# mikemey/cellcomm

Measured on NVIDIA B200. Metric: BiGAN train cells/sec, higher is better.
Workload: dtype bf16

## Files before the change

cellcomm_b200/csrc/gemm_sm100.cu:

```cuda
#include <cuda.h>

#include <mutex>
#include <unordered_map>

#include "common.cuh"

namespace cc {

constexpr int BM = 128;
constexpr int BK = 64;
constexpr int UMMA_K = 16;
constexpr int MAX_SEG = CC_GEMM_MAX_SEG;

struct EpiParams {
  int M, N;
  float alpha;
  const float* bias;
  int act;
  const bf16* dact_y;
  long long ld_dact;
  int dact;
  bf16* out16;
  long long ld16;
  int beta16;
// ... 884 lines not shown
      const int nkb_u = unit_nkb(u);
      int seg = 0, kb_in_seg = unit_kb0(u);
      while (seg < p.nseg - 1 && kb_in_seg >= p.kblocks[seg]) {
        kb_in_seg -= p.kblocks[seg];
        ++seg;
      }
      for (int i = 0; i < nkb_u; ++i, ++it) {
        const int s = it % STAGES;
        const uint32_t ph = (it / STAGES) & 1u;
        mbar_wait(empty_bar(s), ph ^ 1u, 11);
        if (elect_one()) {
          const uint32_t a_dst = smem_base + s * STAGE_BYTES;
          const uint32_t b_dst = a_dst + A_BYTES;
          const int k0 = kb_in_seg * BK;
          mbar_expect_tx(full_bar(s), p.stage_tx);
          if (RMS_DIRECT && A_MN && B_MN && keep != 0) {
#pragma unroll
            for (int j = 0; j < BM / 64; ++j)
              tma_load_2d_pol(a_dst + j * (64 * BK * 2), &maps.a[seg], full_bar(s), m0 + 64 * j, k0,
                              keep);
#pragma unroll
            for (int j = 0; j < BN / 64; ++j) {
              if (j >= p.b_boxes) continue;
              if (CLUSTER == 2) {
                if ((j & 1) == rank)
                  tma_load_2d_mc_pol(b_dst + j * (64 * BK * 2), &maps.b[seg], full_bar(s),
                                     n0 + 64 * j, k0, (uint16_t)3, keep);
              } else {
                tma_load_2d_pol(b_dst + j * (64 * BK * 2), &maps.b[seg], full_bar(s), n0 + 64 * j,
                                k0, keep);
              }
            }
          } else if (A_MN) {
#pragma unroll
            for (int j = 0; j < BM / 64; ++j)
              tma_load_2d(a_dst + j * (64 * BK * 2), &maps.a[seg], full_bar(s), m0 + 64 * j, k0);
          } else {
            tma_load_2d(a_dst, &maps.a[seg], full_bar(s), k0, m0);
          }
          if (RMS_DIRECT && A_MN && B_MN && keep != 0) {
          } else if (CLUSTER == 2) {
            if (B_MN) {
#pragma unroll
              for (int j = 0; j < BN / 64; ++j)
                if (j < p.b_boxes && (j & 1) == rank)
                  tma_load_2d_mc(b_dst + j * (64 * BK * 2), &maps.b[seg], full_bar(s), n0 + 64 * j,
                                 k0, (uint16_t)3);
            } else {
              tma_load_2d_mc(b_dst + rank * p.b_half_rows * (BK * 2), &maps.b[seg], full_bar(s), k0,
                             n0 + rank * p.b_half_rows, (uint16_t)3);
            }
          } else if (B_MN) {
#pragma unroll
            for (int j = 0; j < BN / 64; ++j)
              if (j < p.b_boxes)
                tma_load_2d(b_dst + j * (64 * BK * 2), &maps.b[seg], full_bar(s), n0 + 64 * j, k0);
          } else {
            tma_load_2d(b_dst, &maps.b[seg], full_bar(s), k0, n0);
          }
        }
        __syncwarp();
        if (++kb_in_seg >= p.kblocks[seg] && seg < p.nseg - 1) {
          kb_in_seg = 0;
          ++seg;
        }
      }
    }
  } else if (warp == 1) {
    uint32_t it = 0, tl = 0;
    for (int u = unit0; (!PAIR || rank == 0) && u < num_units; u += unit_step, ++tl) {
      const uint32_t acc = tl & 1u, aph = (tl >> 1) & 1u;
      mbar_wait(tempty_bar(acc), aph ^ 1u, 12);
      tcgen05_fence_after();
      const uint32_t d_tmem = tmem_acc + acc * BN;
      const int nkb = unit_nkb(u);
      for (int i = 0; i < nkb; ++i, ++it) {
        const int s = it % STAGES;
        const uint32_t ph = (it / STAGES) & 1u;
        mbar_wait(full_bar(s), ph, 13);
        tcgen05_fence_after();
        if (elect_one()) {
          const uint32_t a_src = smem_base + s * STAGE_BYTES;
          const uint32_t b_src = a_src + A_BYTES;
#pragma unroll
          for (int k = 0; k < BK / UMMA_K; ++k) {
            const uint64_t adesc = p.adesc_hi | (uint64_t)(((a_src + k * p.a_kstep) & 0x3FFFFu) >> 4);
            const uint64_t bdesc = p.bdesc_hi | (uint64_t)(((b_src + k * p.b_kstep) & 0x3FFFFu) >> 4);
            if (PAIR) umma_bf16_pair(d_tmem, adesc, bdesc, p.idesc, (i > 0 || k > 0) ? 1u : 0u);
            else umma_bf16(d_tmem, adesc, bdesc, p.idesc, (i > 0 || k > 0) ? 1u : 0u);
          }
          if (PAIR) {
            umma_commit_pair(empty_bar(s), (uint16_t)3);
            if (i == nkb - 1) umma_commit_pair(tfull_bar(acc), (uint16_t)3);
          } else {
            if (CLUSTER == 2) umma_commit_mc(empty_bar(s), (uint16_t)3);
            else umma_commit(empty_bar(s));
            if (i == nkb - 1) umma_commit(tfull_bar(acc));
          }
        }
        __syncwarp();
      }
    }
  } else {
    const int q = warp & 3;
    const int ew = warp - 2;
    constexpr int COLS_PER_WARP = BN / (EPI_WARPS / 4);
    const int col_lo = (ew >> 2) * COLS_PER_WARP;
    uint32_t tl = 0;
    for (int u = unit0; u < num_units; u += unit_step, ++tl) {
      const int m0 = unit_m0(u), n0 = unit_n0(u);
      const uint32_t acc = tl & 1u, aph = (tl >> 1) & 1u;
      mbar_wait(tfull_bar(acc), aph, 14);
      tcgen05_fence_after();
      const uint32_t t_row = tmem_acc + ((uint32_t)(q * 32) << 16) + acc * BN;
      if (m0 < p.epi.M) {
#pragma unroll 1
        for (int c = col_lo; c < col_lo + COLS_PER_WARP; c += 32) {
          if (c >= p.bn_eff || n0 + c >= p.epi.N) break;
          uint32_t raw[32];
          tmem_ld32(t_row + (uint32_t)c, raw);
          tmem_ld_wait();
          if constexpr (RMS_DIRECT) rms_blocked_chunk(p.epi, lane, m0 + q * 32, n0 + c, raw);
          else epilogue_chunk<MATH>(p.epi, epi_stage + ew * (32 * EPI_LD), lane, m0 + q * 32, n0 + c, raw,
                                    (long long)unit_split(u) * p.partial_stride);
        }
      }
      tcgen05_fence_before();
      __syncwarp();
      if (lane == 0) {
        if (PAIR) mbar_arrive_cluster(mapa_cluster(tempty_bar(acc), 0));
        else mbar_arrive(tempty_bar(acc));
      }
    }
  }
  tcgen05_fence_before();
  __syncthreads();
  if (CLUSTER == 2) cluster_sync_all();
  if (warp == 1) {
    if (PAIR)
      asm volatile("tcgen05.dealloc.cta_group::2.sync.aligned.b32 %0, %1;" ::"r"(tmem_acc),
                   "r"(TMEM_COLS)
                   : "memory");
    else
      asm volatile("tcgen05.dealloc.cta_group::1.sync.aligned.b32 %0, %1;" ::"r"(tmem_acc),
                   "r"(TMEM_COLS)
                   : "memory");
  }
}

}
#include "wgrad_rmsprop_kernel.cuh"
namespace cc {

__global__ void splitk_finalize_kernel(const EpiParams e, const float* __restrict__ partial,
                                       long long partial_ld, long long partial_stride, int splits) {
  const int groups = (e.N + 3) / 4;
  const long long idx = (long long)blockIdx.x * blockDim.x + threadIdx.x;
  if (idx >= (long long)e.M * groups) return;
  const int r = (int)(idx / groups);
  const int c0 = (int)(idx % groups) * 4;
  const float* src = partial + (long long)r * partial_ld + c0;
  float4 a = make_float4(0.f, 0.f, 0.f, 0.f);
  for (int s0 = 0; s0 < splits; s0 += 8) {
    float4 q[8];
#pragma unroll
    for (int u = 0; u < 8; ++u)
      q[u] = (s0 + u < splits)
                 ? __ldcs(reinterpret_cast<const float4*>(src + (long long)(s0 + u) * partial_stride))
                 : make_float4(0.f, 0.f, 0.f, 0.f);
#pragma unroll
    for (int u = 0; u < 8; ++u) {
      if (s0 + u < splits) {
        a.x += q[u].x;
        a.y += q[u].y;
        a.z += q[u].z;
        a.w += q[u].w;
      }
    }
  }
  float v[4] = {a.x, a.y, a.z, a.w};
  const int ncols = min(4, e.N - c0);
#pragma unroll
  for (int j = 0; j < 4; ++j) {
    float x = v[j] * e.alpha;
    if (e.bias != nullptr && j < ncols) x += __ldg(e.bias + c0 + j);
    if (e.act == CC_ACT_SIGMOID) x = sigmoidf_(x);
    else if (e.act == CC_ACT_RELU) x = fmaxf(x, 0.f);
    v[j] = x;
  }
  if (e.dact != 0) {
    const bf16* yrow = e.dact_y + (long long)r * e.ld_dact + c0;
#pragma unroll
    for (int j = 0; j < 4; ++j) {
      if (j < ncols) {
        const float y = bf2f(yrow[j]);
        v[j] *= (e.dact == CC_ACT_SIGMOID) ? y * (1.f - y) : (y > 0.f ? 1.f : 0.f);
      }
    }
  }
  if (e.out32 != nullptr) {
    float* o = e.out32 + (long long)r * e.ld32 + c0;
    if (ncols == 4 && (((uintptr_t)o) & 15) == 0 && !e.beta32) {
      *reinterpret_cast<float4*>(o) = make_float4(v[0], v[1], v[2], v[3]);
    } else {
#pragma unroll
      for (int j = 0; j < 4; ++j)
        if (j < ncols) o[j] = e.beta32 ? o[j] + v[j] : v[j];
    }
  }
  if (e.out16 != nullptr) {
    bf16* o = e.out16 + (long long)r * e.ld16 + c0;
    if (ncols == 4 && (((uintptr_t)o) & 7) == 0 && !e.beta16) {
      __nv_bfloat162 p0 = __floats2bfloat162_rn(v[0], v[1]);
      __nv_bfloat162 p1 = __floats2bfloat162_rn(v[2], v[3]);
      uint2 u;
      u.x = *reinterpret_cast<uint32_t*>(&p0);
      u.y = *reinterpret_cast<uint32_t*>(&p1);
      *reinterpret_cast<uint2*>(o) = u;
    } else {
#pragma unroll
      for (int j = 0; j < 4; ++j)
        if (j < ncols) o[j] = f2bf(e.beta16 ? bf2f(o[j]) + v[j] : v[j]);
    }
    if (e.out16_lo != nullptr) {
      bf16* l = e.out16_lo + (long long)r * e.ld16_lo + c0;
#pragma unroll
      for (int j = 0; j < 4; ++j)
        if (j < ncols) l[j] = f2bf(v[j] - bf2f(f2bf(v[j])));
    }
  }
}

typedef CUresult (*PFN_encodeTiled)(CUtensorMap*, CUtensorMapDataType, cuuint32_t, void*,
                                    const cuuint64_t*, const cuuint64_t*, const cuuint32_t*,
                                    const cuuint32_t*, CUtensorMapInterleave, CUtensorMapSwizzle,
                                    CUtensorMapL2promotion, CUtensorMapFloatOOBfill);

static PFN_encodeTiled get_encode_fn() {
  static PFN_encodeTiled fn = nullptr;
  static std::once_flag once;
  std::call_once(once, [] {
    void* ptr = nullptr;
    cudaDriverEntryPointQueryResult qres;
    if (cudaGetDriverEntryPoint("cuTensorMapEncodeTiled", &ptr, cudaEnableDefault, &qres) ==
            cudaSuccess &&
        qres == cudaDriverEntryPointSuccess)
      fn = (PFN_encodeTiled)ptr;
  });
  return fn;
}

struct MapKey {
  const void* ptr;
  uint64_t inner, outer, ld;
  uint32_t box_inner, box_outer;
  uint32_t kind;
  bool operator==(const MapKey& o) const {
    return ptr == o.ptr && inner == o.inner && outer == o.outer && ld == o.ld &&
           box_inner == o.box_inner && box_outer == o.box_outer && kind == o.kind;
  }
};
struct MapKeyHash {
  size_t operator()(const MapKey& k) const {
    uint64_t h = (uint64_t)(uintptr_t)k.ptr * 0x9E3779B97F4A7C15ull;
    h ^= k.inner + 0x9E3779B97F4A7C15ull + (h << 6) + (h >> 2);
    h ^= k.outer + 0x9E3779B97F4A7C15ull + (h << 6) + (h >> 2);
    h ^= k.ld + 0x9E3779B97F4A7C15ull + (h << 6) + (h >> 2);
    h ^= ((uint64_t)k.box_inner << 32 | k.box_outer) + 0x9E3779B97F4A7C15ull + (h << 6) + (h >> 2);
    h ^= k.kind + 0x9E3779B97F4A7C15ull + (h << 6) + (h >> 2);
    return (size_t)h;
  }
};

enum MapKind : uint32_t {
  MAP_BF16_SW128 = 0,
  MAP_F32_SW128 = 1,
  MAP_BF16_SW64 = 2,
  MAP_F32_SW128_L2_256 = 3
};

static int make_map_kind(CUtensorMap* out, const void* ptr, uint64_t inner, uint64_t outer,
                         uint64_t ld, uint32_t box_inner, uint32_t box_outer, MapKind kind) {
  static std::mutex mu;
  static std::unordered_map<MapKey, CUtensorMap, MapKeyHash> cache;
  MapKey key{ptr, inner, outer, ld, box_inner, box_outer, (uint32_t)kind};
  {
    std::lock_guard<std::mutex> g(mu);
    auto it = cache.find(key);
    if (it != cache.end()) {
      *out = it->second;
      return 0;
    }
  }
  const bool f32 = kind == MAP_F32_SW128 || kind == MAP_F32_SW128_L2_256;
  const uint64_t esize = f32 ? 4 : 2;
  PFN_encodeTiled enc = get_encode_fn();
  CC_REQUIRE(enc != nullptr, "cuTensorMapEncodeTiled is unavailable (no CUDA driver?)");
  CC_REQUIRE(((uintptr_t)ptr & 15) == 0, "cc_gemm: operand base %p is not 16-byte aligned", ptr);
  CC_REQUIRE((ld * esize) % 16 == 0, "cc_gemm: operand ld=%llu is not a multiple of 16 bytes",
             (unsigned long long)ld);
  CC_REQUIRE(inner > 0 && outer > 0, "cc_gemm: empty operand");
  cuuint64_t dims[2] = {inner, outer};
  cuuint64_t strides[1] = {ld * esize};
  cuuint32_t box[2] = {box_inner, box_outer};
  cuuint32_t estr[2] = {1, 1};
  CUresult r = enc(out,
                   f32 ? CU_TENSOR_MAP_DATA_TYPE_FLOAT32 : CU_TENSOR_MAP_DATA_TYPE_BFLOAT16,
                   2, const_cast<void*>(ptr), dims, strides, box, estr,
                   CU_TENSOR_MAP_INTERLEAVE_NONE,
                   kind == MAP_BF16_SW64 ? CU_TENSOR_MAP_SWIZZLE_64B : CU_TENSOR_MAP_SWIZZLE_128B,
                   (kind == MAP_BF16_SW128 || kind == MAP_F32_SW128_L2_256)
                       ? CU_TENSOR_MAP_L2_PROMOTION_L2_256B
                       : CU_TENSOR_MAP_L2_PROMOTION_L2_128B,
                   CU_TENSOR_MAP_FLOAT_OOB_FILL_NONE);
  CC_REQUIRE(r == CUDA_SUCCESS,
             "cuTensorMapEncodeTiled failed (%d) ptr=%p inner=%llu outer=%llu ld=%llu box=%ux%u",
             (int)r, ptr, (unsigned long long)inner, (unsigned long long)outer,
             (unsigned long long)ld, box_inner, box_outer);
  {
    std::lock_guard<std::mutex> g(mu);
    if (cache.size() > (1u << 16)) cache.clear();
    cache.emplace(key, *out);
  }
  return 0;
}

static int make_map(CUtensorMap* out, const void* ptr, uint64_t inner, uint64_t outer, uint64_t ld,
                    uint32_t box_inner, uint32_t box_outer) {
  return make_map_kind(out, ptr, inner, outer, ld, box_inner, box_outer, MAP_BF16_SW128);
}

static uint64_t desc_hi(uint32_t lbo_bytes, uint32_t sbo_bytes) {
  uint64_t d = 0;
  d |= (uint64_t)((lbo_bytes >> 4) & 0x3FFF) << 16;
  d |= (uint64_t)((sbo_bytes >> 4) & 0x3FFF) << 32;
  d |= (uint64_t)1 << 46;
  d |= (uint64_t)2 << 61;
  return d;
}

static int env_int(const char* name, int dflt) {
  const char* v = getenv(name);
  return v ? atoi(v) : dflt;
}

struct GemmEnv {
  int sms;
  int bn;
  int splits;
  int persistent;
  int cluster;
  int rms_cluster;
  int bn_eff;
  int mn_lbo;
  int mn_sbo;
  int mn_kstep;
  int k_lbo;
  int k_sbo;
  int rms_cs;
  int rms_warps;
  int rms_nfast;
  int rms_tma;
  int rms_p16_tma;
  int rms_interleave;
  int rms_pair;
  int pair;
  int rms_l2_256;
  int rms_keep;
  int persistent_splitk;
};
static GemmEnv g_env;
static std::atomic<int> g_env_state{0};
static std::mutex g_env_mu;
static int g_num_sms = 0;

static const GemmEnv& gemm_env() {
  if (g_env_state.load(std::memory_order_acquire) == 0) {
    std::lock_guard<std::mutex> lock(g_env_mu);
    GemmEnv e;
    e.sms = env_int("CC_GEMM_SMS", 0);
    e.bn = env_int("CC_GEMM_BN", 0);
    e.splits = env_int("CC_GEMM_SPLITS", 0);
    e.persistent = env_int("CC_GEMM_PERSISTENT", 1);
    e.cluster = env_int("CC_GEMM_CLUSTER", 2);
    e.rms_cluster = env_int("CC_GEMM_RMS_CLUSTER", -1);
    e.bn_eff = env_int("CC_GEMM_BN_EFF", 0);
    e.mn_lbo = env_int("CC_GEMM_MN_LBO", 64 * BK * 2);
    e.mn_sbo = env_int("CC_GEMM_MN_SBO", 1024);
    e.mn_kstep = env_int("CC_GEMM_MN_KSTEP", UMMA_K * 128);
    e.k_lbo = env_int("CC_GEMM_K_LBO", 16);
    e.k_sbo = env_int("CC_GEMM_K_SBO", 1024);
    e.rms_cs = env_int("CC_GEMM_RMS_CS", 1);
    e.rms_warps = env_int("CC_GEMM_RMS_WARPS", 8);
    e.rms_nfast = env_int("CC_GEMM_RMS_NFAST", -1);
    e.rms_tma = env_int("CC_GEMM_RMS_TMA", -1);
    e.rms_p16_tma = env_int("CC_GEMM_RMS_P16_TMA", 0);
    e.rms_interleave = env_int("CC_GEMM_RMS_INTERLEAVE", 1);
    e.rms_pair = env_int("CC_GEMM_RMS_PAIR", 0);
    e.pair = env_int("CC_GEMM_PAIR", 0);
    e.rms_l2_256 = env_int("CC_GEMM_RMS_L2_256", 0);
    e.rms_keep = env_int("CC_GEMM_RMS_KEEP_OPERANDS", 0);
    e.persistent_splitk = env_int("CC_GEMM_PERSISTENT_SPLITK", 1);
    g_env = e;
    g_env_state.store(1, std::memory_order_release);
  }
  return g_env;
}

template <int BN, int STAGES>
static constexpr size_t smem_bytes() {
  return (size_t)STAGES * (BM * BK * 2 + BN * BK * 2) + 8 * (2 * STAGES + 2) + 1024;
}

template <int BN, int STAGES, bool A_MN, bool B_MN>
static int launch_cfg(const TmaMaps& maps, const GemmParams& p, dim3 grid, cudaStream_t st) {
  auto kern = gemm_tcgen05_kernel<BN, STAGES, A_MN, B_MN>;
  static bool attr_set = false;
  constexpr size_t smem = smem_bytes<BN, STAGES>();
  if (!attr_set) {
    CC_CHECK_CUDA(cudaFuncSetAttribute(kern, cudaFuncAttributeMaxDynamicSharedMemorySize, (int)smem));
    attr_set = true;
  }
  kern<<<grid, 128, smem, st>>>(maps, p);
  CC_CHECK_LAUNCH();
  return 0;
}

template <int BN, int STAGES>
static int launch_major(const TmaMaps& maps, const GemmParams& p, dim3 grid, bool a_mn, bool b_mn,
                        cudaStream_t st) {
  if (!a_mn && b_mn) return launch_cfg<BN, STAGES, false, true>(maps, p, grid, st);
  if (!a_mn && !b_mn) return launch_cfg<BN, STAGES, false, false>(maps, p, grid, st);
  if (a_mn && b_mn) return launch_cfg<BN, STAGES, true, true>(maps, p, grid, st);
  return launch_cfg<BN, STAGES, true, false>(maps, p, grid, st);
}

template <int BN, int STAGES, int EPI_WARPS, bool PAIR = false, bool RMS_DIRECT = false>
static constexpr size_t smem_bytes_persistent() {
  return (size_t)STAGES * (BM * BK * 2 + (PAIR ? BN / 2 : BN) * BK * 2) + 8 * (2 * STAGES + 6) + 16 +
         (RMS_DIRECT ? 0 : EPI_WARPS * 32 * EPI_LD * 4) + 1024;
}

template <int BN, int STAGES, bool A_MN, bool B_MN, bool MATH, int EPI_WARPS, bool N_FAST, int CLUSTER,
          bool PAIR = false, bool RMS_DIRECT = false>
static int launch_persistent_one(const TmaMaps& maps, const GemmParams& p, int mt, int nt,
                                 int num_sms, cudaStream_t st) {
  auto kern = gemm_tcgen05_persistent_kernel<BN, STAGES, A_MN, B_MN, MATH, EPI_WARPS, N_FAST, CLUSTER,
                                             PAIR, RMS_DIRECT>;
  static bool attr_set = false;
  static int max_ctas = 0;
  constexpr size_t smem = smem_bytes_persistent<BN, STAGES, EPI_WARPS, PAIR, RMS_DIRECT>();
  static_assert(smem <= 232448, "shared memory per CTA");
  constexpr int threads = 64 + 32 * EPI_WARPS;
  if (!attr_set) {
    CC_CHECK_CUDA(cudaFuncSetAttribute(kern, cudaFuncAttributeMaxDynamicSharedMemorySize, (int)smem));
    max_ctas = num_sms;
    if (CLUSTER > 1) {
      cudaLaunchConfig_t q{};
      q.gridDim = dim3((unsigned)(num_sms / CLUSTER * CLUSTER));
      q.blockDim = dim3(threads);
      q.dynamicSmemBytes = smem;
      cudaLaunchAttribute qa[1];
      qa[0].id = cudaLaunchAttributeClusterDimension;
      qa[0].val.clusterDim.x = CLUSTER;
      qa[0].val.clusterDim.y = 1;
      qa[0].val.clusterDim.z = 1;
      q.attrs = qa;
      q.numAttrs = 1;
      int nclusters = 0;
      CC_CHECK_CUDA(cudaOccupancyMaxActiveClusters(&nclusters, kern, &q));
      CC_REQUIRE(nclusters >= 1, "cc_gemm: no %d-CTA cluster fits on this device", CLUSTER);
      if (nclusters * CLUSTER < max_ctas) max_ctas = nclusters * CLUSTER;
    }
    attr_set = true;
  }
  const int units = ((mt + CLUSTER - 1) / CLUSTER) * nt * (p.psplits > 1 ? p.psplits : 1);
  int grid = units * CLUSTER < max_ctas ? units * CLUSTER : max_ctas / CLUSTER * CLUSTER;
  cudaLaunchConfig_t cfg{};
  cfg.gridDim = dim3((unsigned)grid);
  cfg.blockDim = dim3(threads);
  cfg.dynamicSmemBytes = smem;
  cfg.stream = st;
  cudaLaunchAttribute attr[1];
  attr[0].id = cudaLaunchAttributeClusterDimension;
  attr[0].val.clusterDim.x = CLUSTER;
  attr[0].val.clusterDim.y = 1;
  attr[0].val.clusterDim.z = 1;
  cfg.attrs = attr;
  cfg.numAttrs = 1;
  CC_CHECK_CUDA(cudaLaunchKernelEx(&cfg, kern, maps, p, mt, nt));
  count_launch();
  return 0;
}

template <int BN, int STAGES, int EPI_WARPS>
static constexpr int pair_stages() {
  return BN == 256 ? (EPI_WARPS == 8 ? 5 : 6) : STAGES;
}

template <int BN, int STAGES, bool A_MN, bool B_MN, bool MATH, int EPI_WARPS = 4, bool N_FAST = false>
static int launch_persistent_cfg(const TmaMaps& maps, const GemmParams& p, int mt, int nt,
                                 int num_sms, cudaStream_t st) {
  if (BN == 256 && p.cluster == 2 && p.pair)
    return launch_persistent_one<BN, pair_stages<BN, STAGES, EPI_WARPS>(), A_MN, B_MN, MATH, EPI_WARPS,
                                 N_FAST, 2, BN == 256>(maps, p, mt, nt, num_sms, st);
  if (p.cluster == 2)
    return launch_persistent_one<BN, STAGES, A_MN, B_MN, MATH, EPI_WARPS, N_FAST, 2>(maps, p, mt, nt, num_sms, st);
  return launch_persistent_one<BN, STAGES, A_MN, B_MN, MATH, EPI_WARPS, N_FAST, 1>(maps, p, mt, nt, num_sms, st);
}

template <int BN, int STAGES, bool MATH>
static int launch_persistent_m(const TmaMaps& maps, const GemmParams& p, int mt, int nt,
                               int num_sms, bool a_mn, bool b_mn, cudaStream_t st) {
  if (!a_mn && b_mn) return launch_persistent_cfg<BN, STAGES, false, true, MATH>(maps, p, mt, nt, num_sms, st);
  if (!a_mn && !b_mn) return launch_persistent_cfg<BN, STAGES, false, false, MATH>(maps, p, mt, nt, num_sms, st);
  if (a_mn && b_mn) return launch_persistent_cfg<BN, STAGES, true, true, MATH>(maps, p, mt, nt, num_sms, st);
  return launch_persistent_cfg<BN, STAGES, true, false, MATH>(maps, p, mt, nt, num_sms, st);
}

template <int BN, int STAGES>
static int launch_persistent(const TmaMaps& maps, const GemmParams& p, int mt, int nt, int num_sms,
                             bool a_mn, bool b_mn, cudaStream_t st) {
  const EpiParams& e = p.epi;
  const bool math = e.alpha != 1.f || e.bias != nullptr || e.act != 0 || e.dact != 0;
  if (math) return launch_persistent_m<BN, STAGES, true>(maps, p, mt, nt, num_sms, a_mn, b_mn, st);
  return launch_persistent_m<BN, STAGES, false>(maps, p, mt, nt, num_sms, a_mn, b_mn, st);
}

template <bool N_FAST, int CLUSTER, bool PAIR = false>
static int launch_rms_tma(const RmsMaps& maps, const GemmParams& p, int mt, int nt, int num_sms,
                          cudaStream_t st) {
  static_assert(!PAIR || CLUSTER == 2, "the CTA pair is a cluster of two");
  void (*kern)(const RmsMaps, const GemmParams, const int, const int);
  if (PAIR) kern = wgrad_rmsprop_pair_kernel<N_FAST>;
  else kern = wgrad_rmsprop_tma_kernel<N_FAST, CLUSTER>;
  static bool attr_set = false;
  static int max_ctas = 0;
  constexpr size_t smem = PAIR ? RMSP_SMEM_BYTES : RMS_SMEM_BYTES;
  constexpr int threads = 64 + 32 * RMS_EPI_WARPS;
  if (!attr_set) {
    CC_CHECK_CUDA(cudaFuncSetAttribute(kern, cudaFuncAttributeMaxDynamicSharedMemorySize, (int)smem));
    max_ctas = num_sms;
    if (CLUSTER > 1) {
      cudaLaunchConfig_t q{};
      q.gridDim = dim3((unsigned)(num_sms / CLUSTER * CLUSTER));
      q.blockDim = dim3(threads);
      q.dynamicSmemBytes = smem;
      cudaLaunchAttribute qa[1];
      qa[0].id = cudaLaunchAttributeClusterDimension;
      qa[0].val.clusterDim.x = CLUSTER;
      qa[0].val.clusterDim.y = 1;
      qa[0].val.clusterDim.z = 1;
      q.attrs = qa;
      q.numAttrs = 1;
      int nclusters = 0;
      CC_CHECK_CUDA(cudaOccupancyMaxActiveClusters(&nclusters, kern, &q));
      CC_REQUIRE(nclusters >= 1, "cc_gemm: no %d-CTA cluster fits on this device", CLUSTER);
      if (nclusters * CLUSTER < max_ctas) max_ctas = nclusters * CLUSTER;
    }
    attr_set = true;
  }
  const int units = ((mt + CLUSTER - 1) / CLUSTER) * nt;
  int grid = units * CLUSTER < max_ctas ? units * CLUSTER : max_ctas / CLUSTER * CLUSTER;
  cudaLaunchConfig_t cfg{};
  cfg.gridDim = dim3((unsigned)grid);
  cfg.blockDim = dim3(threads);
  cfg.dynamicSmemBytes = smem;
  cfg.stream = st;
  cudaLaunchAttribute attr[1];
  attr[0].id = cudaLaunchAttributeClusterDimension;
  attr[0].val.clusterDim.x = CLUSTER;
  attr[0].val.clusterDim.y = 1;
  attr[0].val.clusterDim.z = 1;
  cfg.attrs = attr;
  cfg.numAttrs = 1;
  CC_CHECK_CUDA(cudaLaunchKernelEx(&cfg, kern, maps, p, mt, nt));
  count_launch();
  return 0;
}

int gemm_impl(const cc_gemm_desc* d, cudaStream_t st) {
  const GemmEnv& ENV = gemm_env();
  CC_REQUIRE(d != nullptr, "cc_gemm: null descriptor");
  CC_REQUIRE(d->M > 0 && d->N > 0, "cc_gemm: empty output %dx%d", d->M, d->N);
  CC_REQUIRE(d->nseg >= 1 && d->nseg <= MAX_SEG, "cc_gemm: nseg=%d out of range", d->nseg);
  CC_REQUIRE(d->out16 != nullptr || d->out32 != nullptr || d->rms_p32 != nullptr,
             "cc_gemm: no output");
  CC_REQUIRE(d->rms_p32 == nullptr || (d->rms_ms != nullptr && d->rms_mom != nullptr),
             "cc_gemm: fused RMSprop needs ms and mom");
  CC_REQUIRE(d->route_world >= 0 && d->route_world <= CC_PEER_MAX, "cc_gemm: route_world=%d",
             d->route_world);
  CC_REQUIRE(d->out16_lo == nullptr || (d->out16 != nullptr && d->beta16 == 0),
             "cc_gemm: out16_lo needs a plain out16 (the high-order term)");
  if (d->rms_blocked) {
    CC_REQUIRE(d->rms_p32 != nullptr && d->a_mn_major && d->b_mn_major && d->N > 128 &&
                   d->alpha == 1.f && d->bias == nullptr && d->act == 0 && d->dact_y == nullptr &&
                   d->out16 == nullptr && d->beta32 == 0 && d->route_world == 0 &&
                   d->force_splits <= 1 && (d->force_bn == 0 || d->force_bn == 256),
               "cc_gemm: rms_blocked is for plain weight-gradient GEMMs (X^T dZ, N > 128)");
    CC_REQUIRE(d->rms_row0 >= 0 && (d->rms_ld & 31) == 0 &&
                   ((((uintptr_t)d->rms_p32) | ((uintptr_t)d->rms_ms) | ((uintptr_t)d->rms_mom) |
                     ((uintptr_t)d->rms_p16) | ((uintptr_t)d->rms_p16_lo) | ((uintptr_t)d->out32)) & 15) == 0 &&
                   (d->out32 == nullptr || (d->ld32 & 3) == 0),
               "cc_gemm: rms_blocked needs 16-byte aligned blocks, rms_ld %% 32 == 0 (rms_ld=%lld)",
               (long long)d->rms_ld);
  }
  CC_REQUIRE(d->rms_p16_lo == nullptr || d->rms_blocked,
             "cc_gemm: rms_p16_lo is written by the blocked fused-optimiser epilogue only");
  if (d->route_world > 0) {
    CC_REQUIRE(d->out32 != nullptr && d->beta32 == 0 && d->workspace == nullptr &&
                   d->rms_p32 == nullptr,
               "cc_gemm: a routed output needs a plain fp32 output without split-K");
    CC_REQUIRE(d->route_shard > 0 && (d->route_shard & 7) == 0 && d->route_shard < (1ll << 32) &&
                   d->route_off0 >= 0 && (d->route_off0 & 3) == 0,
               "cc_gemm: route_shard=%lld route_off0=%lld", (long long)d->route_shard,
               (long long)d->route_off0);
    for (int q = 0; q < d->route_world; ++q)
      CC_REQUIRE(d->route_base[q] != nullptr, "cc_gemm: route_base[%d] is null", q);
  }
  if (g_num_sms == 0) {
    int dev = 0;
    CC_CHECK_CUDA(cudaGetDevice(&dev));
    CC_CHECK_CUDA(cudaDeviceGetAttribute(&g_num_sms, cudaDevAttrMultiProcessorCount, dev));
    const int cap = ENV.sms;
    if (cap >= 2 && cap < g_num_sms) g_num_sms = cap / 2 * 2;
  }
  const bool a_mn = d->a_mn_major != 0, b_mn = d->b_mn_major != 0;

  int bn = d->force_bn ? d->force_bn : ENV.bn;
  if (bn == 0) bn = (d->N > 128) ? 256 : 128;
  CC_REQUIRE(bn == 128 || bn == 256, "cc_gemm: BN=%d unsupported", bn);

  GemmParams p{};
  TmaMaps maps;
  memset(&maps, 0, sizeof(maps));
  p.nseg = d->nseg;
  int total = 0;
  for (int s = 0; s < d->nseg; ++s) {
    CC_REQUIRE(d->k[s] > 0, "cc_gemm: segment %d has k=%d", s, d->k[s]);
    p.kblocks[s] = (d->k[s] + BK - 1) / BK;
    total += p.kblocks[s];
  }
  p.total_kblocks = total;

  const int mt = (d->M + BM - 1) / BM;
  int nt = (d->N + bn - 1) / bn;
  int splits = 1;
  const long long Mpad = (long long)mt * BM, Npad = (long long)nt * bn;
  if (d->workspace != nullptr && d->rms_p32 == nullptr) {
    int want = d->force_splits ? d->force_splits : ENV.splits;
    if (want == 0) {
      const int tiles = mt * nt;
      if (2 * tiles <= g_num_sms && total >= 8) {
        want = (2 * g_num_sms) / tiles;
        if (want < 1) want = 1;
        if (want > total / 4) want = total / 4;
      } else {
        want = 1;
      }
    }
    if (want > total) want = total;
    const long long cap = d->workspace_elems / (Mpad * Npad);
    if (want > cap) want = (int)cap;
    if (want >= 2) splits = want;
  }
  p.kb_per_split = (total + splits - 1) / splits;
  splits = (total + p.kb_per_split - 1) / p.kb_per_split;
  if (splits >= 2) {
    p.partial = d->workspace;
    p.partial_ld = Npad;
    p.partial_stride = Mpad * Npad;
  } else {
    p.partial = nullptr;
    p.kb_per_split = total;
    splits = 1;
  }
  const bool psk = splits >= 2 && ENV.persistent != 0 && ENV.persistent_splitk != 0;
  const bool persistent =
      (splits == 1 || psk) && (ENV.persistent != 0 || d->rms_p32 != nullptr ||
                               d->route_world > 0);

  const bool rms_cluster = ENV.rms_cluster < 0 ? total > 8 : ENV.rms_cluster != 0;
  p.cluster = (persistent && mt >= 2 && ENV.cluster == 2 &&
               (d->rms_p32 == nullptr || rms_cluster)) ? 2 : 1;
  int bn_eff = bn;
  if (persistent && bn == 256 && d->rms_p32 == nullptr && splits == 1) {
    const int forced = ENV.bn_eff;
    if (forced >= 32 && forced <= 256 && forced % 32 == 0) {
      bn_eff = forced;
    } else {
      long long best = -1;
      const int mu = (mt + p.cluster - 1) / p.cluster, slots = g_num_sms / p.cluster;
      for (int cand = 256; cand >= 128; cand -= 64) {
        const long long units = (long long)mu * ((d->N + cand - 1) / cand);
        const long long cost = ((units + slots - 1) / slots) * (cand + 128);
        if (best < 0 || cost < best) {
          best = cost;
          bn_eff = cand;
        }
      }
    }
    nt = (d->N + bn_eff - 1) / bn_eff;
  }
  p.bn_eff = bn_eff;
  p.b_boxes = (bn_eff + 63) / 64;
  p.b_half_rows = bn_eff / 2;
  p.stage_tx = (unsigned)(BM * BK * 2 + (b_mn ? p.b_boxes * 64 * BK * 2 : bn_eff * BK * 2));
  p.pair = (p.cluster == 2 && bn == 256 && ENV.pair != 0 && splits == 1 &&
            (b_mn ? bn_eff % 128 == 0 : bn_eff % 32 == 0)) ? 1 : 0;
  if (p.pair) {
    p.b_boxes = bn_eff / 128;
    p.stage_tx = (unsigned)(BM * BK * 2 + (bn_eff / 2) * BK * 2);
  }

  for (int s = 0; s < d->nseg; ++s) {
    int rc;
    if (a_mn)
      rc = make_map(&maps.a[s], d->a[s], (uint64_t)d->M, (uint64_t)d->k[s], (uint64_t)d->lda[s], 64, BK);
    else
      rc = make_map(&maps.a[s], d->a[s], (uint64_t)d->k[s], (uint64_t)d->M, (uint64_t)d->lda[s], BK, BM);
    if (rc) return rc;
    if (b_mn)
      rc = make_map(&maps.b[s], d->b[s], (uint64_t)d->N, (uint64_t)d->k[s], (uint64_t)d->ldb[s], 64, BK);
    else
      rc = make_map(&maps.b[s], d->b[s], (uint64_t)d->k[s], (uint64_t)d->N, (uint64_t)d->ldb[s], BK,
                    (uint32_t)(persistent ? (p.cluster == 2 ? bn_eff / 2 : bn_eff) : bn));
    if (rc) return rc;
  }

  const uint32_t mn_lbo = (uint32_t)ENV.mn_lbo;
  const uint32_t mn_sbo = (uint32_t)ENV.mn_sbo;
  const uint32_t mn_kstep = (uint32_t)ENV.mn_kstep;
  const uint32_t k_lbo = (uint32_t)ENV.k_lbo;
  const uint32_t k_sbo = (uint32_t)ENV.k_sbo;
  p.adesc_hi = a_mn ? desc_hi(mn_lbo, mn_sbo) : desc_hi(k_lbo, k_sbo);
  p.bdesc_hi = b_mn ? desc_hi(mn_lbo, mn_sbo) : desc_hi(k_lbo, k_sbo);
  p.a_kstep = a_mn ? mn_kstep : UMMA_K * 2;
  p.b_kstep = b_mn ? mn_kstep : UMMA_K * 2;
  p.idesc = (1u << 4) | (1u << 7) | (1u << 10) | ((a_mn ? 1u : 0u) << 15) |
            ((b_mn ? 1u : 0u) << 16) | ((uint32_t)((persistent ? bn_eff : bn) >> 3) << 17) |
            ((uint32_t)(((persistent && p.pair) ? 2 * BM : BM) >> 4) << 24);

  EpiParams& e = p.epi;
  e.M = d->M;
  e.N = d->N;
  e.alpha = d->alpha;
  e.bias = d->bias;
  e.act = d->act;
  e.dact_y = (const bf16*)d->dact_y;
  e.ld_dact = d->ld_dact;
  e.dact = d->dact_y ? d->dact : 0;
  e.out16 = (bf16*)d->out16;
  e.ld16 = d->ld16;
  e.beta16 = d->beta16;
  e.out16_lo = (bf16*)d->out16_lo;
  e.ld16_lo = d->ld16_lo;
  e.out32 = d->out32;
  e.ld32 = d->ld32;
  e.beta32 = d->beta32;
  e.rms_p32 = d->rms_p32;
  e.rms_ms = d->rms_ms;
  e.rms_mom = d->rms_mom;
  e.rms_p16 = (bf16*)d->rms_p16;
  e.rms_ld = d->rms_ld;
  e.rms_lr = d->rms_lr;
  e.rms_rho = d->rms_rho;
  e.rms_momentum = d->rms_momentum;
  e.rms_eps = d->rms_eps;
  e.rms_cs = (ENV.rms_cs ? 1 : 0) | (ENV.rms_l2_256 ? 8 : 0);
  e.rms_blocked = d->rms_blocked;
  e.rms_row0 = d->rms_row0;
  e.rms_p16lo = d->rms_blocked ? (bf16*)d->rms_p16_lo : nullptr;
  e.rms_keep_operands = ENV.rms_keep;
  e.route_world = d->route_world;
  e.route_shard = (unsigned)d->route_shard;
  e.route_off0 = d->route_off0;
  for (int q = 0; q < CC_PEER_MAX; ++q)
    e.route_base[q] = q < d->route_world ? d->route_base[q] : nullptr;

  if (persistent) {
// ... 118 lines not shown
```

Before: 58550.

## Add mma.sync small-GEMM path with split-K for small shapes

Adds a cp.async and ldmatrix based mma.sync kernel with 64x64 tiles, a 4-stage pipeline and optional split-K, and routes small or skinny GEMMs to it by default instead of the tcgen05/TMA kernel. The goal is to avoid the fixed setup cost and poor SM fill of the large-tile UMMA path on small problems. It also moves the split-K finalize epilogue into a shared templated helper. The risk is that the shape heuristic sends some GEMMs to a slower legacy tensor-core path.

```diff
diff --git a/cellcomm_b200/csrc/gemm_sm100.cu b/cellcomm_b200/csrc/gemm_sm100.cu
--- a/cellcomm_b200/csrc/gemm_sm100.cu
+++ b/cellcomm_b200/csrc/gemm_sm100.cu
@@ -1060,6 +1060,67 @@
 #include "wgrad_rmsprop_kernel.cuh"
 namespace cc {
 
+template <int NC>
+__device__ __forceinline__ void epilogue_store_cols(const EpiParams& e, int r, int c0, float (&v)[NC]) {
+  const int ncols = min(NC, e.N - c0);
+#pragma unroll
+  for (int j = 0; j < NC; ++j) {
+    float x = v[j] * e.alpha;
+    if (e.bias != nullptr && j < ncols) x += __ldg(e.bias + c0 + j);
+    if (e.act == CC_ACT_SIGMOID) x = sigmoidf_(x);
+    else if (e.act == CC_ACT_RELU) x = fmaxf(x, 0.f);
+    v[j] = x;
+  }
+  if (e.dact != 0) {
+    const bf16* yrow = e.dact_y + (long long)r * e.ld_dact + c0;
+#pragma unroll
+    for (int j = 0; j < NC; ++j) {
+      if (j < ncols) {
+        const float y = bf2f(yrow[j]);
+        v[j] *= (e.dact == CC_ACT_SIGMOID) ? y * (1.f - y) : (y > 0.f ? 1.f : 0.f);
+      }
+    }
+  }
+  if (e.out32 != nullptr) {
+    float* o = e.out32 + (long long)r * e.ld32 + c0;
+    if (ncols == NC && (((uintptr_t)o) & (4 * NC - 1)) == 0 && !e.beta32) {
+      if constexpr (NC == 4)
+        *reinterpret_cast<float4*>(o) = make_float4(v[0], v[1], v[2], v[3]);
+      else
+        *reinterpret_cast<float2*>(o) = make_float2(v[0], v[1]);
+    } else {
+#pragma unroll
+      for (int j = 0; j < NC; ++j)
+        if (j < ncols) o[j] = e.beta32 ? o[j] + v[j] : v[j];
+    }
+  }
+  if (e.out16 != nullptr) {
+    bf16* o = e.out16 + (long long)r * e.ld16 + c0;
+    if (ncols == NC && (((uintptr_t)o) & (2 * NC - 1)) == 0 && !e.beta16) {
+      __nv_bfloat162 p0 = __floats2bfloat162_rn(v[0], v[1]);
+      if constexpr (NC == 4) {
+        __nv_bfloat162 p1 = __floats2bfloat162_rn(v[2], v[3]);
+        uint2 u;
+        u.x = *reinterpret_cast<uint32_t*>(&p0);
+        u.y = *reinterpret_cast<uint32_t*>(&p1);
+        *reinterpret_cast<uint2*>(o) = u;
+      } else {
+        *reinterpret_cast<__nv_bfloat162*>(o) = p0;
+      }
+    } else {
+#pragma unroll
+      for (int j = 0; j < NC; ++j)
+        if (j < ncols) o[j] = f2bf(e.beta16 ? bf2f(o[j]) + v[j] : v[j]);
+    }
+    if (e.out16_lo != nullptr) {
+      bf16* l = e.out16_lo + (long long)r * e.ld16_lo + c0;
+#pragma unroll
+      for (int j = 0; j < NC; ++j)
+        if (j < ncols) l[j] = f2bf(v[j] - bf2f(f2bf(v[j])));
+    }
+  }
+}
+
 __global__ void splitk_finalize_kernel(const EpiParams e, const float* __restrict__ partial,
                                        long long partial_ld, long long partial_stride, int splits) {
   const int groups = (e.N + 3) / 4;
@@ -1087,56 +1148,163 @@
     }
   }
   float v[4] = {a.x, a.y, a.z, a.w};
-  const int ncols = min(4, e.N - c0);
-#pragma unroll
-  for (int j = 0; j < 4; ++j) {
-    float x = v[j] * e.alpha;
-    if (e.bias != nullptr && j < ncols) x += __ldg(e.bias + c0 + j);
-    if (e.act == CC_ACT_SIGMOID) x = sigmoidf_(x);
-    else if (e.act == CC_ACT_RELU) x = fmaxf(x, 0.f);
-    v[j] = x;
-  }
-  if (e.dact != 0) {
-    const bf16* yrow = e.dact_y + (long long)r * e.ld_dact + c0;
-#pragma unroll
-    for (int j = 0; j < 4; ++j) {
-      if (j < ncols) {
-        const float y = bf2f(yrow[j]);
-        v[j] *= (e.dact == CC_ACT_SIGMOID) ? y * (1.f - y) : (y > 0.f ? 1.f : 0.f);
-      }
-    }
-  }
-  if (e.out32 != nullptr) {
-    float* o = e.out32 + (long long)r * e.ld32 + c0;
-    if (ncols == 4 && (((uintptr_t)o) & 15) == 0 && !e.beta32) {
-      *reinterpret_cast<float4*>(o) = make_float4(v[0], v[1], v[2], v[3]);
+  epilogue_store_cols<4>(e, r, c0, v);
+}
+
+constexpr int SG_BM = 64, SG_BN = 64, SG_BK = 32, SG_STAGES = 4, SG_THREADS = 128;
+constexpr int SG_TILE = 64 * (SG_BK + 8);
+
+struct SmallGemmParams {
+  EpiParams epi;
+  const bf16* a[MAX_SEG];
+  const bf16* b[MAX_SEG];
+  long long lda[MAX_SEG], ldb[MAX_SEG];
+  int k[MAX_SEG];
+  int kblocks[MAX_SEG];
+  int nseg, total_kblocks, kb_per_split;
+  float* partial;
+  long long partial_ld, partial_stride;
+};
+
+__device__ __forceinline__ void cp_async16(uint32_t dst, const void* src, int bytes) {
+  asm volatile("cp.async.cg.shared.global [%0], [%1], 16, %2;" ::"r"(dst), "l"(src), "r"(bytes)
+               : "memory");
+}
+__device__ __forceinline__ void ldsm_x4(uint32_t addr, uint32_t (&r)[4]) {
+  asm volatile("ldmatrix.sync.aligned.m8n8.x4.shared.b16 {%0, %1, %2, %3}, [%4];"
+               : "=r"(r[0]), "=r"(r[1]), "=r"(r[2]), "=r"(r[3])
+               : "r"(addr));
+}
+__device__ __forceinline__ void ldsm_x4_t(uint32_t addr, uint32_t (&r)[4]) {
+  asm volatile("ldmatrix.sync.aligned.m8n8.x4.trans.shared.b16 {%0, %1, %2, %3}, [%4];"
+               : "=r"(r[0]), "=r"(r[1]), "=r"(r[2]), "=r"(r[3])
+               : "r"(addr));
+}
+__device__ __forceinline__ void mma_bf16_16816(float (&c)[4], const uint32_t (&a)[4], uint32_t b0,
+                                               uint32_t b1) {
+  asm volatile(
+      "mma.sync.aligned.m16n8k16.row.col.f32.bf16.bf16.f32 {%0, %1, %2, %3}, {%4, %5, %6, %7}, "
+      "{%8, %9}, {%0, %1, %2, %3};"
+      : "+f"(c[0]), "+f"(c[1]), "+f"(c[2]), "+f"(c[3])
+      : "r"(a[0]), "r"(a[1]), "r"(a[2]), "r"(a[3]), "r"(b0), "r"(b1));
+}
+
+template <bool MN_MAJOR>
+__device__ __forceinline__ void sg_load_tile(uint32_t dst, const bf16* base, long long ld, int i0,
+                                             int outer_n, int k0, int kn) {
+#pragma unroll
+  for (int q = 0; q < 2; ++q) {
+    const int c = threadIdx.x + q * SG_THREADS;
+    int valid, sidx;
+    long long off;
+    if (MN_MAJOR) {
+      const int row = c >> 3, col = (c & 7) * 8;
+      const int gk = k0 + row, gi = i0 + col;
+      valid = gk < kn ? min(max(outer_n - gi, 0), 8) : 0;
+      off = (long long)gk * ld + gi;
+      sidx = row * (SG_BM + 8) + col;
     } else {
-#pragma unroll
-      for (int j = 0; j < 4; ++j)
-        if (j < ncols) o[j] = e.beta32 ? o[j] + v[j] : v[j];
-    }
-  }
-  if (e.out16 != nullptr) {
-    bf16* o = e.out16 + (long long)r * e.ld16 + c0;
-    if (ncols == 4 && (((uintptr_t)o) & 7) == 0 && !e.beta16) {
-      __nv_bfloat162 p0 = __floats2bfloat162_rn(v[0], v[1]);
-      __nv_bfloat162 p1 = __floats2bfloat162_rn(v[2], v[3]);
-      uint2 u;
-      u.x = *reinterpret_cast<uint32_t*>(&p0);
-      u.y = *reinterpret_cast<uint32_t*>(&p1);
-      *reinterpret_cast<uint2*>(o) = u;
-    } else {
-#pragma unroll
-      for (int j = 0; j < 4; ++j)
-        if (j < ncols) o[j] = f2bf(e.beta16 ? bf2f(o[j]) + v[j] : v[j]);
-    }
-    if (e.out16_lo != nullptr) {
-      bf16* l = e.out16_lo + (long long)r * e.ld16_lo + c0;
-#pragma unroll
-      for (int j = 0; j < 4; ++j)
-        if (j < ncols) l[j] = f2bf(v[j] - bf2f(f2bf(v[j])));
-    }
-  }
+      const int row = c >> 2, col = (c & 3) * 8;
+      const int gi = i0 + row, gk = k0 + col;
+      valid = gi < outer_n ? min(max(kn - gk, 0), 8) : 0;
+      off = (long long)gi * ld + gk;
+      sidx = row * (SG_BK + 8) + col;
+    }
+    cp_async16(dst + 2u * (uint32_t)sidx, valid > 0 ? (const void*)(base + off) : (const void*)base,
+               valid * 2);
+  }
+}
+
+template <bool A_MN, bool B_MN>
+__global__ void __launch_bounds__(SG_THREADS) gemm_small_kernel(const SmallGemmParams p) {
+  __shared__ __align__(128) bf16 sa[SG_STAGES][SG_TILE];
+  __shared__ __align__(128) bf16 sb[SG_STAGES][SG_TILE];
+  const int M = p.epi.M, N = p.epi.N;
+  const int m0 = blockIdx.y * SG_BM, n0 = blockIdx.x * SG_BN;
+  const int kb_begin = blockIdx.z * p.kb_per_split;
+  const int nkb = min(p.kb_per_split, p.total_kblocks - kb_begin);
+  const int warp = threadIdx.x >> 5, lane = threadIdx.x & 31;
+  const int wm = (warp >> 1) * 32, wn = (warp & 1) * 32;
+
+  int ls = 0, lkb = kb_begin;
+  while (ls < p.nseg - 1 && lkb >= p.kblocks[ls]) lkb -= p.kblocks[ls++];
+  auto load_next = [&](int stage) {
+    const int k0 = lkb * SG_BK, kn = p.k[ls];
+    sg_load_tile<A_MN>(smem_u32(&sa[stage][0]), p.a[ls], p.lda[ls], m0, M, k0, kn);
+    sg_load_tile<B_MN>(smem_u32(&sb[stage][0]), p.b[ls], p.ldb[ls], n0, N, k0, kn);
+    if (++lkb == p.kblocks[ls] && ls < p.nseg - 1) {
+      lkb = 0;
+      ++ls;
+    }
+  };
+
+  float acc[2][4][4];
+#pragma unroll
+  for (int i = 0; i < 2; ++i)
+#pragma unroll
+    for (int j = 0; j < 4; ++j)
+#pragma unroll
+      for (int t = 0; t < 4; ++t) acc[i][j][t] = 0.f;
+
+#pragma unroll
+  for (int s = 0; s < SG_STAGES - 1; ++s) {
+    if (s < nkb) load_next(s);
+    asm volatile("cp.async.commit_group;" ::: "memory");
+  }
+  const int li = lane & 7, lm = lane >> 3;
+  for (int it = 0; it < nkb; ++it) {
+    asm volatile("cp.async.wait_group %0;" ::"n"(SG_STAGES - 2) : "memory");
+    __syncthreads();
+    const int st = it % SG_STAGES;
+    const uint32_t a_s = smem_u32(&sa[st][0]), b_s = smem_u32(&sb[st][0]);
+#pragma unroll
+    for (int kk = 0; kk < SG_BK; kk += 16) {
+      uint32_t af[2][4], bfr[2][4];
+#pragma unroll
+      for (int mi = 0; mi < 2; ++mi) {
+        const int mb = wm + mi * 16;
+        if (A_MN)
+          ldsm_x4_t(a_s + 2u * ((kk + li + (lm >> 1) * 8) * (SG_BM + 8) + mb + (lm & 1) * 8), af[mi]);
+        else
+          ldsm_x4(a_s + 2u * ((mb + (lane & 15)) * (SG_BK + 8) + kk + (lane >> 4) * 8), af[mi]);
+      }
+#pragma unroll
+      for (int nj = 0; nj < 2; ++nj) {
+        const int nb = wn + nj * 16;
+        if (B_MN)
+          ldsm_x4_t(b_s + 2u * ((kk + li + (lm & 1) * 8) * (SG_BN + 8) + nb + (lm >> 1) * 8), bfr[nj]);
+        else
+          ldsm_x4(b_s + 2u * ((nb + li + (lm >> 1) * 8) * (SG_BK + 8) + kk + (lm & 1) * 8), bfr[nj]);
+      }
+#pragma unroll
+      for (int mi = 0; mi < 2; ++mi)
+#pragma unroll
+        for (int ni = 0; ni < 4; ++ni)
+          mma_bf16_16816(acc[mi][ni], af[mi], bfr[ni >> 1][(ni & 1) * 2], bfr[ni >> 1][(ni & 1) * 2 + 1]);
+    }
+    if (it + SG_STAGES - 1 < nkb) load_next((it + SG_STAGES - 1) % SG_STAGES);
+    asm volatile("cp.async.commit_group;" ::: "memory");
+  }
+
+#pragma unroll
+  for (int mi = 0; mi < 2; ++mi)
+#pragma unroll
+    for (int h = 0; h < 2; ++h) {
+      const int r = m0 + wm + mi * 16 + (lane >> 2) + h * 8;
+      if (r >= M) continue;
+#pragma unroll
+      for (int ni = 0; ni < 4; ++ni) {
+        const int c = n0 + wn + ni * 8 + (lane & 3) * 2;
+        if (c >= N) continue;
+        float v[2] = {acc[mi][ni][2 * h], acc[mi][ni][2 * h + 1]};
+        if (p.partial != nullptr) {
+          float* o = p.partial + blockIdx.z * p.partial_stride + (long long)r * p.partial_ld + c;
+          *reinterpret_cast<float2*>(o) = make_float2(v[0], v[1]);
+        } else {
+          epilogue_store_cols<2>(p.epi, r, c, v);
+        }
+      }
+    }
 }
 
 typedef CUresult (*PFN_encodeTiled)(CUtensorMap*, CUtensorMapDataType, cuuint32_t, void*,
@@ -1276,6 +1444,7 @@
   int rms_l2_256;
   int rms_keep;
   int persistent_splitk;
+  int small;
 };
 static GemmEnv g_env;
 static std::atomic<int> g_env_state{0};
@@ -1309,6 +1478,7 @@
     e.rms_l2_256 = env_int("CC_GEMM_RMS_L2_256", 0);
     e.rms_keep = env_int("CC_GEMM_RMS_KEEP_OPERANDS", 0);
     e.persistent_splitk = env_int("CC_GEMM_PERSISTENT_SPLITK", 1);
+    e.small = env_int("CC_GEMM_SMALL", 1);
     g_env = e;
     g_env_state.store(1, std::memory_order_release);
   }
@@ -1487,6 +1657,89 @@
   return 0;
 }
 
+static bool use_small_gemm(const cc_gemm_desc* d, bool any_eligible) {
+  if (d->rms_p32 != nullptr || d->route_world > 0 || d->force_bn != 0 || d->force_splits != 0)
+    return false;
+  long long ktot = 0;
+  for (int s = 0; s < d->nseg; ++s) {
+    ktot += d->k[s];
+    if ((((uintptr_t)d->a[s]) & 15) || (((uintptr_t)d->b[s]) & 15) || (d->lda[s] & 7) ||
+        (d->ldb[s] & 7))
+      return false;
+  }
+  if (d->a_mn_major) {
+    const long long mn = (long long)d->M * d->N;
+    if (d->M > 2048 || d->N > 2048 || mn > (1ll << 19)) return false;
+    return any_eligible || (d->b_mn_major && mn <= (1ll << 17) && ktot >= 1024);
+  }
+  if (d->N > 512 || ktot > 2048) return false;
+  return any_eligible || (d->b_mn_major && ktot <= 320);
+}
+
+static int launch_small(const cc_gemm_desc* d, cudaStream_t st) {
+  SmallGemmParams p;
+  memset(&p, 0, sizeof(p));
+  EpiParams& e = p.epi;
+  e.M = d->M;
+  e.N = d->N;
+  e.alpha = d->alpha;
+  e.bias = d->bias;
+  e.act = d->act;
+  e.dact_y = (const bf16*)d->dact_y;
+  e.ld_dact = d->ld_dact;
+  e.dact = d->dact_y ? d->dact : 0;
+  e.out16 = (bf16*)d->out16;
+  e.ld16 = d->ld16;
+  e.beta16 = d->beta16;
+  e.out16_lo = (bf16*)d->out16_lo;
+  e.ld16_lo = d->ld16_lo;
+  e.out32 = d->out32;
+  e.ld32 = d->ld32;
+  e.beta32 = d->beta32;
+  p.nseg = d->nseg;
+  for (int s = 0; s < d->nseg; ++s) {
+    CC_REQUIRE(d->k[s] > 0, "cc_gemm: segment %d has k=%d", s, d->k[s]);
+    p.a[s] = (const bf16*)d->a[s];
+    p.b[s] = (const bf16*)d->b[s];
+    p.lda[s] = d->lda[s];
+    p.ldb[s] = d->ldb[s];
+    p.k[s] = d->k[s];
+    p.kblocks[s] = (d->k[s] + SG_BK - 1) / SG_BK;
+    p.total_kblocks += p.kblocks[s];
+  }
+  const int mt = (d->M + SG_BM - 1) / SG_BM, nt = (d->N + SG_BN - 1) / SG_BN;
+  int splits = 1;
+  const long long pld = (d->N + 3) / 4 * 4;
+  if (d->a_mn_major && d->workspace != nullptr) {
+    splits = min(2 * g_num_sms / (mt * nt), p.total_kblocks / 8);
+    const long long cap = d->workspace_elems / ((long long)d->M * pld);
+    if (splits > cap) splits = (int)cap;
+    if (splits < 1) splits = 1;
+  }
+  p.kb_per_split = (p.total_kblocks + splits - 1) / splits;
+  splits = (p.total_kblocks + p.kb_per_split - 1) / p.kb_per_split;
+  if (splits >= 2) {
+    p.partial = d->workspace;
+    p.partial_ld = pld;
+    p.partial_stride = (long long)d->M * pld;
+  }
+  const dim3 grid((unsigned)nt, (unsigned)mt, (unsigned)splits);
+  const bool a_mn = d->a_mn_major != 0, b_mn = d->b_mn_major != 0;
+  if (a_mn && b_mn) gemm_small_kernel<true, true><<<grid, SG_THREADS, 0, st>>>(p);
+  else if (a_mn) gemm_small_kernel<true, false><<<grid, SG_THREADS, 0, st>>>(p);
+  else if (b_mn) gemm_small_kernel<false, true><<<grid, SG_THREADS, 0, st>>>(p);
+  else gemm_small_kernel<false, false><<<grid, SG_THREADS, 0, st>>>(p);
+  CC_CHECK_LAUNCH();
+  if (splits >= 2) {
+    const long long work = (long long)d->M * ((d->N + 3) / 4);
+    const int threads = 256;
+    splitk_finalize_kernel<<<(unsigned)((work + threads - 1) / threads), threads, 0, st>>>(
+        e, p.partial, p.partial_ld, p.partial_stride, splits);
+    CC_CHECK_LAUNCH();
+  }
+  return 0;
+}
+
 int gemm_impl(const cc_gemm_desc* d, cudaStream_t st) {
   const GemmEnv& ENV = gemm_env();
   CC_REQUIRE(d != nullptr, "cc_gemm: null descriptor");
@@ -1534,6 +1787,8 @@
     if (cap >= 2 && cap < g_num_sms) g_num_sms = cap / 2 * 2;
   }
   const bool a_mn = d->a_mn_major != 0, b_mn = d->b_mn_major != 0;
+
+  if (ENV.small != 0 && use_small_gemm(d, ENV.small == 2)) return launch_small(d, st);
 
   int bn = d->force_bn ? d->force_bn : ENV.bn;
   if (bn == 0) bn = (d->N > 128) ? 256 : 128;
```

Measured after the change: 59140 (median of 6 runs). +1.0%, better.
